# agiger/GPR

Measured on AMD Instinct MI355X. Metric: GP fits/sec (kernel build + Cholesky + solve), N=16384 d=32 fp64, higher is better.
Workload: dtype f64

## Files before the change

gpr_amd/csrc/k_pt_ops.h:

```cpp
#pragma once
#include "k_handoff.h"
#include "k_mma.h"

namespace gprx {
namespace pt {

using namespace mm;
using ho::ld_agent;
using ho::ld_sys;
using ho::ld_uni;
using ho::local_sync;
using ho::publish;
using ho::publish2;
using ho::st_agent;
using ho::st_sys;
using ho::wait_until;
using ho::wave_id;

template <typename T, bool UPDATE, int MAP = 0>
__device__ __forceinline__ void tile_gemm(T* __restrict__ C, int64_t ldc, const T* __restrict__ A, int64_t lda,
                                          const T* __restrict__ B, int64_t ldb, int K, bool lower, T* smem,
                                          const int t, bool tri = false, const uint64_t* Bpan = nullptr) {
    typedef Mfma<T> Tr;
    typedef typename Tr::acc_t acc_t;
    const int lane = t & 63, w = t >> 6;
    int wr, wc;
    wave_block<MAP>(w, wr, wc);
    const int lr = lane & 15, lk = lane >> 4;
    const bool active = !(lower && wr == 0 && wc >= 2);
    T cv[2][4][4];
    if (UPDATE && active) {
#pragma unroll
        for (int x = 0; x < 2; x++)
#pragma unroll
            for (int reg = 0; reg < 4; reg++) {
                const int jl = wc * 32 + x * 16 + Tr::orow(lk, reg);
                const T* ccol = C + (int64_t)jl * ldc;
#pragma unroll
                for (int y = 0; y < 4; y++) cv[x][y][reg] = ccol[wr * 64 + y * 16 + lr];
            }
    }
    acc_t acc[2][4];
    tile_mma<T, MAP>(acc, A, lda, B, ldb, K, !active ? 0 : (tri ? 32 * (wc + 1) : K), smem, t, Bpan);
    if (!active) return;
#pragma unroll
    for (int x = 0; x < 2; x++) {
#pragma unroll
        for (int reg = 0; reg < 4; reg++) {
            const int jl = wc * 32 + x * 16 + Tr::orow(lk, reg);
            T* ccol = C + (int64_t)jl * ldc;
#pragma unroll
            for (int y = 0; y < 4; y++) {
                const int il = wr * 64 + y * 16 + lr;
                if (UPDATE)
                    st_sc1(ccol + il, (lower && il < jl) ? cv[x][y][reg] : cv[x][y][reg] - acc[x][y][reg]);
                else if (!lower || il >= jl)
                    st_sc1(ccol + il, acc[x][y][reg]);
            }
        }
    }
}

template <typename T>
__device__ __forceinline__ void tile_trsm(T* C, int64_t ldc, const T* A, int64_t lda,
                                          const T* __restrict__ B, int64_t ldb, T* smem, const int t) {
    typedef Mfma<T> Tr;
    const int lane = t & 63, w = t >> 6, lr = lane & 15, lk = lane >> 4;
    typename Tr::acc_t acc[2][4];
    mm::tile_mma_trirows<T>(acc, A, lda, B, ldb, smem, t);
#pragma unroll
    for (int x = 0; x < 2; x++)
#pragma unroll
        for (int y = 0; y < 4; y++)
#pragma unroll
            for (int reg = 0; reg < 4; reg++)
                st_sc1(C + (int64_t)(16 * (4 * x + y) + Tr::orow(lk, reg)) * ldc + 16 * w + lr, acc[x][y][reg]);
}

template <typename T>
__device__ __forceinline__ void tile_gemm_rows16(T* __restrict__ C, int64_t ldc, const T* __restrict__ A, int64_t lda,
                                                 const T* __restrict__ B, int64_t ldb, int K, T* smem, const int t) {
    typedef Mfma<T> Tr;
    const int lane = t & 63, w = t >> 6, lr = lane & 15, lk = lane >> 4;
    T cv[4];
#pragma unroll
    for (int reg = 0; reg < 4; reg++) cv[reg] = C[(int64_t)(16 * w + Tr::orow(lk, reg)) * ldc + lr];
    typename Tr::acc_t acc;
    mm::tile_mma_rows16<T>(acc, A, lda, B, ldb, K, smem, t);
#pragma unroll
    for (int reg = 0; reg < 4; reg++) st_sc1(C + (int64_t)(16 * w + Tr::orow(lk, reg)) * ldc + lr, cv[reg] - acc[reg]);
}

template <typename T>
__device__ __forceinline__ void tile_gemm_tall(T* __restrict__ C, int64_t ldc, const T* __restrict__ A, int64_t lda,
                                               const T* __restrict__ B, int64_t ldb, int K, T* smem, const int t) {
    typedef Mfma<T> Tr;
    typedef typename Tr::acc_t acc_t;
    const int lane = t & 63, w = t >> 6;
    const int wr = w & 3, wc = w >> 2, lr = lane & 15, lk = lane >> 4;
    acc_t acc[4][4];
    mm::tile_mma_tall<T, 1>(acc, A, lda, B, ldb, K, smem, t, C, ldc);
#pragma unroll
    for (int x = 0; x < 4; x++)
#pragma unroll
        for (int reg = 0; reg < 4; reg++) {
            T* ccol = C + (int64_t)(64 * wc + 16 * x + Tr::orow(lk, reg)) * ldc;
#pragma unroll
            for (int y = 0; y < 4; y++) st_sc1(ccol + 64 * wr + 16 * y + lr, -acc[x][y][reg]);
        }
}

}
}
```

gpr_amd/csrc/k_ptiles.hip:

```cpp
#include "gprx_dist.h"
#include "gprx_internal.h"
#include "k_handoff.h"
#include "k_pairs.h"
#include "k_pt_diag.h"
#include "k_pt_dist.h"
#include "k_pt_ops.h"
#include "k_pt_split.h"
#include "pt_sched.h"

#include <algorithm>
#include <cstring>
#include <cstdlib>
#include <map>
#include <mutex>
#include <tuple>

namespace gprx {
namespace pt {

template <typename T, int V>
__global__ __launch_bounds__(NT) void diag_bench_kernel(T* A, int64_t ld, T* Linv, int* info, long long* prof,
                                                        int reps) {
    extern __shared__ __attribute__((aligned(16))) unsigned char smem_raw[];
    long long acc[5] = {0, 0, 0, 0, 0};
    long long ph[8] = {0, 0, 0, 0, 0, 0, 0, 0};
    for (int r = 0; r < reps; r++) {
        const long long t0 = wall_clock64();
        if (V == 0) diag_factor_rank8<T>(A + (int64_t)r * DB * ld, ld, Linv, info, 0, smem_raw, threadIdx.x, nullptr, ph);
        else if (V == 1) diag_factor_blocked<T>(A + (int64_t)r * DB * ld, ld, Linv, info, 0, smem_raw, threadIdx.x, ph);
        else diag_factor_la<T>(A + (int64_t)r * DB * ld, ld, Linv, info, 0, smem_raw, threadIdx.x, ph);
        __syncthreads();
        const long long t1 = wall_clock64();
        acc[0] += ph[0];
        acc[1] += ph[1];
        acc[2] += ph[2];
        acc[3] += ph[3];
        acc[4] += t1 - t0;
    }
    if (threadIdx.x == 0) {
        for (int u = 0; u < 5; u++) prof[u] = acc[u];
        for (int u = 0; u < 3; u++) prof[5 + u] = ph[4 + u];
    }
}

template <typename T>
void launch_diag_bench(int variant, T* A, int64_t ld, T* Linv, int* info, long long* prof, int reps, hipStream_t s) {
    const size_t lds = diag_lds<T>() + 64;
    auto go = [&](auto kfn) {
        GPRX_HIP(hipFuncSetAttribute((const void*)kfn, hipFuncAttributeMaxDynamicSharedMemorySize, (int)lds));
        hipLaunchKernelGGL(kfn, dim3(1), dim3(NT), lds, s, A, ld, Linv, info, prof, reps);
    };
    if (variant == 0 || !std::is_same<T, double>::value) go(diag_bench_kernel<T, 0>);
    else if (variant == 1) go(diag_bench_kernel<T, 1>);
    else go(diag_bench_kernel<T, 2>);
    GPRX_HIP(hipGetLastError());
}
template void launch_diag_bench<double>(int, double*, int64_t, double*, int*, long long*, int, hipStream_t);
template void launch_diag_bench<float>(int, float*, int64_t, float*, int*, long long*, int, hipStream_t);

template <typename T>
constexpr size_t pt_lds_bytes() {
    return gemm_lds<T>() > diag_lds<T>() ? gemm_lds<T>() : diag_lds<T>();
}
static_assert(tall_lds<double>() <= pt_lds_bytes<double>() && tall_lds<float>() <= pt_lds_bytes<float>(),
              "the paired update's ring exceeds the LDS of the launch");

template <typename T>
struct Args {
    T* A;
    int64_t ld;
    T* Linv;
    const int4* tasks;
    int ntasks;
    int nc;
    int nv;
    int* ctl;
    int* lcnt;
    int* ver;
    int* info;
    long long tlimit;
    int* dbg;
    int variant;
    long long* trace;
    long long* xt;
    const TileBuild<T>* tb;
    const PtDist<T>* dist;
    int split;
    T* pbuf;
    int* tflag;
    int lab_rows;
};
constexpr int LAB_NARROW = 16;


template <typename T, bool DIST>
__device__ bool wait_inputs(const Args<T>& a, int type, int i, int j, int b0, int nb) {
    const int* vp;
    int vwant;
    const int* vp2;
    int vwant2;
    const int* lp1;
    int lwant1;
    const int* lp2;
    int lwant2;
    const unsigned* rp = nullptr;
    int rn = 0;
    unsigned ep = 0;
    const int* lp3 = nullptr;
    if (type == T_TPART) {
        vp = a.ver + (int64_t)i * a.nv + (i - 1);
        vwant = i - 1;
        vp2 = vp;
        vwant2 = vwant;
        lp1 = a.lcnt + i;
        lwant1 = 0;
        lp2 = lp1;
        lwant2 = 0;
    } else if (type == T_DIAGX && i > 0 && a.split) {
        vp = a.ver + (int64_t)i * a.nv + i;
        vwant = i - 1;
        vp2 = vp;
        vwant2 = vwant;
        lp1 = a.lcnt + i;
        lwant1 = 0;
        lp2 = lp1;
        lwant2 = 0;
    } else if (type == T_DIAGX && i == 0) {
        vp = a.ver;
        vwant = 0;
        vp2 = vp;
        vwant2 = 0;
        lp1 = a.lcnt;
        lwant1 = 0;
        lp2 = lp1;
        lwant2 = 0;
    } else if (type == T_BUILD) {
        return true;
    } else if (type == T_DIAGX) {
        vp = a.ver + (int64_t)i * a.nv + (i - 1);
        vwant = i - 1;
        vp2 = a.ver + (int64_t)i * a.nv + i;
        vwant2 = i - 1;
        lp1 = a.lcnt + (i - 1);
        lwant1 = i;
        lp2 = lp1;
        lwant2 = lwant1;
        if constexpr (DIST) {
            const PtDist<T>& D = *a.dist;
            if (__builtin_amdgcn_readfirstlane(D.loc[i - 1]) < 0) {
                lp1 = lp2 = a.lcnt + i;
                lwant1 = lwant2 = 0;
                rp = dist_flags(D, D.r) + dist_f_linv(D.nr, D.nc) + (i - 1);
                rn = 1;
                ep = D.ep;
            }
        }
    } else if (!DIST && type == T_UPD2) {
        vp = a.ver + (int64_t)i * a.nv + j;
        vwant = b0;
        vp2 = a.ver + (int64_t)(i + 1) * a.nv + j;
        vwant2 = b0;
        lp1 = a.lcnt + i;
        lwant1 = b0 + nb;
        lp2 = a.lcnt + j;
        lwant2 = b0 + nb;
        lp3 = a.lcnt + i + 1;
    } else if (type == T_TRSM) {
        vp = a.ver + (int64_t)i * a.nv + j;
        vwant = j;
        vp2 = vp;
        vwant2 = vwant;
        lp1 = a.lcnt + j;
        lwant1 = j + 1;
        lp2 = lp1;
        lwant2 = lwant1;
        if constexpr (DIST) {
            const PtDist<T>& D = *a.dist;
            if (__builtin_amdgcn_readfirstlane(D.loc[j]) < 0) {
                lp1 = lp2 = a.lcnt + i;
                lwant1 = lwant2 = 0;
                rp = dist_flags(D, D.r) + dist_f_linv(D.nr, D.nc) + j;
                rn = 1;
                ep = D.ep;
            }
        }
    } else {
        const int jc = DIST ? dist_col(a.dist->nc, j) : j;
        vp = a.ver + (int64_t)i * a.nv + jc;
        vwant = b0;
        vp2 = vp;
        vwant2 = vwant;
        lp1 = a.lcnt + i;
        lwant1 = b0 + nb;
        lp2 = a.lcnt + j;
        lwant2 = b0 + nb;
        if constexpr (DIST) {
            const PtDist<T>& D = *a.dist;
            if (__builtin_amdgcn_readfirstlane(D.loc[j]) < 0) {
                lp2 = lp1;
                rp = dist_flags(D, D.r) + dist_f_tile() + (int64_t)j * D.nc + b0;
                rn = nb;
                ep = D.ep;
            }
        }
    }
    const int lane = threadIdx.x & 63;
    const long long t0 = wall_clock64();
    for (;;) {
        int ok = int(ld_uni(vp) == vwant) & int(ld_uni(vp2) == vwant2) & int(ld_uni(lp1) >= lwant1) &
                 int(ld_uni(lp2) >= lwant2);
        if (!DIST && lp3) ok &= int(ld_uni(lp3) >= lwant1);
        if constexpr (DIST) {
            if (rp) {
                const bool good = lane >= rn || ld_sys(rp + (lane < rn ? lane : 0)) == ep;
                ok &= int(__builtin_amdgcn_readfirstlane((uint32_t)(__ballot(!good) == 0)));
            }
        }
        if (ok) return true;
        if (ld_uni(a.ctl + C_ERR)) return false;
        if (wall_clock64() - t0 > a.tlimit) {
            if constexpr (DIST) {
                int miss = int(ld_uni(vp) != vwant) | (int(ld_uni(vp2) != vwant2) << 1) | (int(ld_uni(lp1) < lwant1) << 2) |
                           (int(ld_uni(lp2) < lwant2) << 3);
                int seen = ld_uni(vp);
                if (rp) {
                    const bool good = lane >= rn || ld_sys(rp + (lane < rn ? lane : 0)) == ep;
                    const unsigned long long bad = __ballot(!good);
                    if (bad) {
                        miss |= 16 | ((int)__builtin_ctzll(bad) << 8);
                        seen = (int)__builtin_amdgcn_readfirstlane(ld_sys(rp + (int)__builtin_ctzll(bad)));
                    }
                }
                if (lane == 0) dist_note_timeout(a.dist->check_err + DIST_TO_REC, 1, type, i, j, b0 | (nb << 16), miss, seen);
            }
            st_agent(a.ctl + C_ERR, 1);
            return false;
        }
        __builtin_amdgcn_s_sleep(2);
    }
}

template <typename T>
__device__ __forceinline__ TpCtx<T> tp_ctx(const Args<T>& a) {
    return TpCtx<T>{a.ctl, a.lcnt, a.tflag, a.pbuf, a.dist, a.tlimit, a.xt, a.nc, a.ver, a.nv};
}
template <typename T>
constexpr size_t pt_lds_ctx_off() {
    return pt_lds_bytes<T>() + 16;
}
template <typename T>
constexpr size_t pt_lds_total() {
    return pt_lds_ctx_off<T>() + sizeof(TpCtx<T>);
}

template <typename T, bool DIST>
__global__ __launch_bounds__(NT) void potrf_tiles_kernel(Args<T> a) {
    extern __shared__ __attribute__((aligned(16))) unsigned char smem_raw[];
    int& s_q = *reinterpret_cast<int*>(smem_raw + pt_lds_bytes<T>());
    int& s_ok = *reinterpret_cast<int*>(smem_raw + pt_lds_bytes<T>() + sizeof(int));
    TpCtx<T>* tpc = reinterpret_cast<TpCtx<T>*>(smem_raw + pt_lds_ctx_off<T>());
    if (threadIdx.x == 0) *tpc = tp_ctx(a);
    T* smem = reinterpret_cast<T*>(smem_raw);
    const int t = threadIdx.x;
    const int wv = wave_id();
    const int64_t ld = a.ld;
    for (;;) {
        if (wv == 0) {
            const int v = __hip_atomic_fetch_add(a.ctl + C_TICKET, (t == 0) ? 1 : 0, __ATOMIC_RELAXED,
                                                 __HIP_MEMORY_SCOPE_AGENT);
            s_q = __builtin_amdgcn_readfirstlane(v);
        }
        __syncthreads();
        const int q = __builtin_amdgcn_readfirstlane(s_q);
        if (q >= a.ntasks) break;
        const long long tr0 = a.trace ? wall_clock64() : 0;
        const int4 tk = a.tasks[q];
        const int type = __builtin_amdgcn_readfirstlane(tk.x & 0xff), nb = __builtin_amdgcn_readfirstlane(tk.x >> 8);
        const int i = __builtin_amdgcn_readfirstlane(tk.y), j = __builtin_amdgcn_readfirstlane(tk.z),
                  b0 = __builtin_amdgcn_readfirstlane(tk.w);
        dbg_mark(a.dbg, q, 1 + 10 * type, i, j);
        if (wv == 0) {
            const bool ok0 = wait_inputs<T, DIST>(a, type, i, j, b0, nb);
            if (ok0 && !(a.variant & 32)) {
                bool remote = false;
                if constexpr (DIST) {
                    const PtDist<T>& D = *a.dist;
                    const int dep = (type == T_DIAGX) ? i - 1 : ((type == T_BUILD || type == T_TPART) ? -1 : j);
                    remote = dep >= 0 && __builtin_amdgcn_readfirstlane(D.loc[dep]) < 0 &&
                             !__builtin_amdgcn_readfirstlane(D.acq_agent);
                }
                if (remote) __builtin_amdgcn_fence(__ATOMIC_ACQUIRE, "");
                else __builtin_amdgcn_fence(__ATOMIC_ACQUIRE, "agent");
                asm volatile("s_waitcnt vmcnt(0)" ::: "memory");
            }
            s_ok = ok0 ? 1 : 0;
        }
        __syncthreads();
        if (!__builtin_amdgcn_readfirstlane(s_ok)) break;
        const long long tr1 = a.trace ? wall_clock64() : 0;
        const long long tc1 = a.trace ? (long long)__builtin_amdgcn_s_memtime() : 0;
        dbg_mark(a.dbg, q, 2 + 10 * type, i, j);
        int tid = t;
        asm volatile("" : "+v"(tid));
        if constexpr (DIST) {
            const PtDist<T>& D = *a.dist;
            bool ok = true;
            if (type == T_TPART) {
                ok = tpart_task<T, true>(tpc, dist_tile(a.A, D, i, i - 1), dist_tile(a.A, D, i, i), DB,
                                         a.Linv + (int64_t)(i - 1) * DB * DB, i, j, smem, s_ok, tid);
            } else if (type == T_BUILD) {
                T* tij = dist_tile(a.A, D, i, j);
                const TileBuild<T>& b = *a.tb;
                const bool bad = pr::build_tile_sum<T, 1, true>(
                    b.Kd, b.FU, b.FV, b.nf, b.Kr, b.Kp, b.hd, tij - (int64_t)i * GT - (int64_t)j * GT * DB, DB, b.n,
                    b.sigma2, (int64_t)i * GT, (int64_t)j * GT, smem, tid);
                if (__builtin_amdgcn_readfirstlane(__any(bad))) atomicOr(a.tb->flag, 1);
                publish(a.ver + (int64_t)i * a.nv + j, 0, false);
            } else if (type == T_UPD) {
                const int lj = __builtin_amdgcn_readfirstlane(D.loc[j]);
                const bool loc = lj >= 0;
                const T* Bop = loc ? dist_tile(a.A, D, j, b0) : nullptr;
                const uint64_t* bp = loc ? nullptr : D.tptr + (int64_t)j * D.nc + b0;
                if (D.check && !loc && wv == 0) dist_check_tags(D, j, b0, nb, 0);
                tile_gemm<T, true>(dist_tile(a.A, D, i, j), DB, dist_tile(a.A, D, i, b0), DB, Bop, DB, nb * GT, i == j,
                                   smem, tid, false, bp);
                publish(a.ver + (int64_t)i * a.nv + dist_col(D.nc, j), b0 + nb, false);
                if (D.check && !loc && wv == 0) dist_check_tags(D, j, b0, nb, 1);
                if (!loc && wv == 0) dist_release(D, b0, nb);
            } else if (type == T_TRSM) {
                T* Cik = dist_tile(a.A, D, i, j);
                tile_trsm<T>(Cik, DB, Cik, DB, a.Linv + (int64_t)j * DB * DB, DB, smem, tid);
                publish(a.lcnt + i, j + 1, false);
                if (i == D.nc) {
                    const unsigned all = ((1u << D.g) - 1u) & ~(1u << D.r);
                    dist_push(Cik, D, all, D.o_z + (int64_t)j * DB * DB * (int64_t)sizeof(T),
                              dist_f_tile() + (int64_t)i * D.nc + j, tid);
                } else {
                    const unsigned cm = dist_consumers(D, i);
                    if (wv == 0) ok = dist_wait_release(a, D, cm, j - D.ww);
                    if (wv == 0) s_ok = ok ? 1 : 0;
                    __syncthreads();
                    ok = __builtin_amdgcn_readfirstlane(s_ok) != 0;
                    if (ok)
                        dist_push(Cik, D, cm, -1, dist_f_tile() + (int64_t)i * D.nc + j, tid,
                                  (int64_t)(j % D.ww) * D.nr + i, (D.ep << 16) | (unsigned)(j + 1));
                }
            } else {
                const int k = i;
                T* Akk = dist_tile(a.A, D, k, k);
                T* Akm = k > 0 ? dist_tile(a.A, D, k, k - 1) : nullptr;
                if (k > 0 && a.split) {
                    if constexpr (diag_la<T>) ok = diagx_split<T>(tpc, k, smem, s_ok, tid);
                    else ok = diagx_split_wait<T>(tpc, k, s_ok);
                    if (!ok) break;
                } else if (diag_la<T> && k > 0) {
                    diagx_ts<T>(Akm, Akk, DB, a.Linv + (int64_t)(k - 1) * DB * DB, a.lcnt + k, k, smem, tid, false);
                } else if (k > 0) {
                    tile_trsm<T>(Akm, DB, Akm, DB, a.Linv + (int64_t)(k - 1) * DB * DB, DB, smem, tid);
                    publish(a.lcnt + k, k, false);
                    tile_gemm<T, true, 2>(Akk, DB, Akm, DB, Akm, DB, GT, true, smem, tid);
                    local_sync();
                }
                diag_factor<T>(Akk, DB, a.Linv + (int64_t)k * DB * DB, a.info, (int64_t)k * DB, smem_raw, tid, a.dbg,
                               nullptr, diag_la<T> && k > 0, a.lcnt + k, k + 1);
                const unsigned cm = k > 0 ? dist_consumers(D, k) : 0u;
                const unsigned all = ((1u << D.g) - 1u) & ~(1u << D.r);
                const int nx = (k + 1 < D.nc) ? __builtin_amdgcn_readfirstlane(D.own[k + 1]) : D.r;
                const unsigned first = (nx != D.r) ? (1u << nx) : 0u;
                if (k > 0) {
                    if (wv == 0) ok = dist_wait_release(a, D, cm, k - 1 - D.ww);
                    if (wv == 0) s_ok = ok ? 1 : 0;
                    __syncthreads();
                    ok = __builtin_amdgcn_readfirstlane(s_ok) != 0;
                }
                const int64_t owin = -1;
                const int64_t olinv = D.o_linv + (int64_t)k * DB * DB * (int64_t)sizeof(T);
                const int64_t tix = (int64_t)((k - 1 + D.ww) % D.ww) * D.nr + k;
                const unsigned tgv = (D.ep << 16) | (unsigned)k;
                if (ok && k > 0)
                    dist_push(Akm, D, cm & first, owin, dist_f_tile() + (int64_t)k * D.nc + (k - 1), tid, tix, tgv);
                if (ok) dist_push(a.Linv + (int64_t)k * DB * DB, D, all & first, olinv, dist_f_linv(D.nr, D.nc) + k, tid);
                if (ok && k > 0)
                    dist_push(Akm, D, cm & ~first, owin, dist_f_tile() + (int64_t)k * D.nc + (k - 1), tid, tix, tgv);
                if (ok) dist_push(a.Linv + (int64_t)k * DB * DB, D, all & ~first, olinv, dist_f_linv(D.nr, D.nc) + k, tid);
            }
            if (!ok) break;
        } else {
        T* Ci = a.A + (int64_t)i * GT;
        if (type == T_TPART) {
            (void)tpart_task<T, false>(tpc, Ci + (int64_t)(i - 1) * GT * ld, Ci + (int64_t)i * GT * ld, ld,
                                       a.Linv + (int64_t)(i - 1) * DB * DB, i, j, smem, s_ok, tid);
        } else if (type == T_BUILD) {
            const TileBuild<T>& b = *a.tb;
            const bool bad = pr::build_tile_sum<T, 1, true>(b.Kd, b.FU, b.FV, b.nf, b.Kr, b.Kp, b.hd, a.A, ld, b.n,
                                                            b.sigma2, (int64_t)i * GT, (int64_t)j * GT, smem, tid);
            if (__builtin_amdgcn_readfirstlane(__any(bad))) atomicOr(a.tb->flag, 1);
            publish(a.ver + (int64_t)i * a.nv + j, 0, false);
        } else if (type == T_UPD) {
            const int64_t oa = (a.variant & 64) ? 0 : (int64_t)i * GT + (int64_t)b0 * GT * ld;
            const int64_t ob = (a.variant & 64) ? GT : (int64_t)j * GT + (int64_t)b0 * GT * ld;
            const int64_t lop = (a.variant & 128) ? 0 : ld;
            if (a.variant & 2) {
            } else if (i == a.nc && a.lab_rows <= LAB_NARROW) {
                tile_gemm_rows16<T>(Ci + (int64_t)j * GT * ld, ld, a.A + oa, lop, a.A + ob, lop, nb * GT, smem, tid);
            } else {
                tile_gemm<T, true>(Ci + (int64_t)j * GT * ld, ld, a.A + oa, lop, a.A + ob, lop, nb * GT, i == j, smem,
                                   tid);
            }
            publish(a.ver + (int64_t)i * a.nv + j, b0 + nb, false);
        } else if (type == T_UPD2) {
            if (!(a.variant & 2))
                tile_gemm_tall<T>(Ci + (int64_t)j * GT * ld, ld, a.A + (int64_t)i * GT + (int64_t)b0 * GT * ld, ld,
                                  a.A + (int64_t)j * GT + (int64_t)b0 * GT * ld, ld, nb * GT, smem, tid);
            publish2(a.ver + (int64_t)i * a.nv + j, a.ver + (int64_t)(i + 1) * a.nv + j, b0 + nb);
        } else if (type == T_TRSM) {
            T* Cik = Ci + (int64_t)j * GT * ld;
            if (!(a.variant & 1))
                tile_trsm<T>(Cik, ld, Cik, ld, a.Linv + (int64_t)j * DB * DB, DB, smem, tid);
            publish(a.lcnt + i, j + 1, false);
        } else {
            const int k = i;
            T* Akk = Ci + (int64_t)k * GT * ld;
            long long dt[4] = {0, 0, 0, 0};
            if (k > 0 && a.split) {
                if constexpr (diag_la<T>) (void)diagx_split<T>(tpc, k, smem, s_ok, tid);
                else (void)diagx_split_wait<T>(tpc, k, s_ok);
                if (a.trace) dt[0] = dt[1] = wall_clock64();
            } else if (diag_la<T> && k > 0) {
                T* Akm = Ci + (int64_t)(k - 1) * GT * ld;
                dt[0] = diagx_ts<T>(Akm, Akk, ld, a.Linv + (int64_t)(k - 1) * DB * DB, a.lcnt + k, k, smem, tid,
                                    a.trace != nullptr);
                dt[1] = dt[0];
            } else if (k > 0) {
                T* Akm = Ci + (int64_t)(k - 1) * GT * ld;
                tile_trsm<T>(Akm, ld, Akm, ld, a.Linv + (int64_t)(k - 1) * DB * DB, DB, smem, tid);
                if (a.trace) dt[0] = wall_clock64();
                publish(a.lcnt + k, k, false);
                if (a.trace) dt[1] = wall_clock64();
                tile_gemm<T, true, 2>(Akk, ld, Akm, ld, Akm, ld, GT, true, smem, tid);
                local_sync();
            }
            if (a.trace) dt[2] = wall_clock64();
            diag_factor<T>(Akk, ld, a.Linv + (int64_t)k * DB * DB, a.info, (int64_t)k * DB, smem_raw, tid, a.dbg,
                           a.trace ? a.trace + 4 * (int64_t)(a.ntasks + a.nc) + 4 * (int64_t)k : nullptr,
                           diag_la<T> && k > 0, a.lcnt + k, k + 1);
            if (a.trace) dt[3] = wall_clock64();
            if (a.trace && wv == 0) {
                long long* dp = a.trace + 4 * (int64_t)a.ntasks + 4 * (int64_t)k;
                for (int u = 0; u < 4; u++) dp[u] = dt[u];
            }
        }
        }
        if (a.trace && wv == 0) {
            long long* tp = a.trace + 4 * (int64_t)q;
            tp[0] = tr0;
            tp[1] = tr1;
            tp[2] = wall_clock64();
            tp[3] = (long long)blockIdx.x | (((long long)__builtin_amdgcn_s_memtime() - tc1) << 16);
        }
    }
    dbg_mark(a.dbg, -1, 9, 0, 0);
    if (wv == 0 && ld_agent(a.ctl + C_ERR)) atomicMin(a.info, -1);
}

}

struct PtState {
    struct Dev {
        int4* list = nullptr;
        int64_t n = 0;
        double est_us = 0;
        bool ident_even = false;
        std::vector<int4> host;
    };
    std::map<std::tuple<int, int, bool, int, bool, int>, Dev> sched;
    int* ctr = nullptr;
    void* pbuf = nullptr;
    size_t ctr_ints = 0;
    int ncu = 0;
    int* dbg = nullptr;
    long long* trace = nullptr;
    int64_t trace_n = 0, trace_nc = 0;
    const std::vector<int4>* last_list = nullptr;
    void* tb = nullptr;
    std::vector<unsigned char> tb_last;
    ~PtState() {
        if (tb) (void)hipFree(tb);
        if (pbuf) (void)hipFree(pbuf);
        if (trace) (void)hipFree(trace);
        if (dbg) (void)hipHostFree(dbg);
        for (auto& kv : sched) (void)hipFree(kv.second.list);
        if (ctr) (void)hipFree(ctr);
    }
};

void pt_state_free(PtState* p) { delete p; }

static PtState* g_pt_state = nullptr;
int64_t pt_trace_copy(int32_t* tasks, long long* times, int64_t max) {
    if (!g_pt_state || !g_pt_state->trace || !g_pt_state->last_list) return 0;
    const int64_t n = std::min<int64_t>(max, g_pt_state->trace_n + 7 * g_pt_state->trace_nc);
    GPRX_HIP(hipDeviceSynchronize());
    GPRX_HIP(hipMemcpy(times, g_pt_state->trace, sizeof(long long) * 4 * n, hipMemcpyDeviceToHost));
    const int64_t nl = std::min<int64_t>(n, (int64_t)g_pt_state->last_list->size());
    std::memcpy(tasks, g_pt_state->last_list->data(), sizeof(int4) * nl);
    return n;
}

static int* g_pt_dbg = nullptr;
static int g_pt_dbg_n = 0;
static std::mutex g_pt_dbg_mu;
int pt_debug_snapshot(int* out, int max_wg) {
    std::lock_guard<std::mutex> lk(g_pt_dbg_mu);
    if (!g_pt_dbg) return 0;
    const int n = std::min(max_wg, g_pt_dbg_n);
    for (int k = 0; k < 4 * n; k++) out[k] = __atomic_load_n(g_pt_dbg + k, __ATOMIC_RELAXED);
    return n;
}
void pt_debug_register(int* dbg, int n) {
    std::lock_guard<std::mutex> lk(g_pt_dbg_mu);
    if (n > 0) {
        g_pt_dbg = dbg;
        g_pt_dbg_n = n;
    } else if (g_pt_dbg == dbg) {
        g_pt_dbg = nullptr;
        g_pt_dbg_n = 0;
    }
}

__global__ void pt_init_counters(int* __restrict__ ctr, int64_t n, int64_t v0, int64_t v1) {
    const int64_t i = (int64_t)blockIdx.x * blockDim.x + threadIdx.x;
    if (i < n) ctr[i] = (i >= v0 && i < v1) ? -1 : 0;
}

__global__ void pt_init_identity_counters(int* __restrict__ lcnt, int* __restrict__ ver, int nc, int nr0, int ni,
                                          int even) {
    const int a = blockIdx.x, j = threadIdx.x;
    if (a >= ni) return;
    if (j == 0) lcnt[nr0 + a] = a;
    const int v = even ? a - (a & 1) : a;
    for (int c = j; c < nc; c += blockDim.x) ver[(int64_t)(nr0 + a) * nc + c] = v;
}

template <typename T>
__global__ void pt_init_identity_rows(T* __restrict__ A, int64_t ld, int64_t row0, int64_t nid, int64_t ncol,
                                      int even) {
    const int64_t r = (int64_t)blockIdx.x * blockDim.x + threadIdx.x;
    const int64_t c = blockIdx.y;
    const int64_t rb = r / GT, c0 = (even ? rb - (rb & 1) : rb) * GT;
    if (r >= nid || c >= ncol || c < c0) return;
    A[row0 + r + c * ld] = (r == c) ? T(1) : T(0);
}

template <typename T>
void potrf_tiles(T* A, int64_t ld, int64_t np, int64_t nrows, T* Linv, int* info, Exec& ex, const TileBuild<T>* build,
                 int ni, bool build_only, int lab_live) {
    using namespace pt;
    if (!ex.pt) ex.pt = new PtState();
    PtState& st = *ex.pt;
    if (st.ncu == 0) {
        int dev = 0;
        GPRX_HIP(hipGetDevice(&dev));
        hipDeviceProp_t prop;
        GPRX_HIP(hipGetDeviceProperties(&prop, dev));
        st.ncu = prop.multiProcessorCount;
    }
    GPRX_REQUIRE(np % DB == 0 && nrows % GT == 0 && nrows >= np, GPRX_ERR_ARG, "potrf_tiles: bad sizes");
    const int nc = (int)(np / DB), nr = (int)(nrows / GT);
    const bool fused = build && build->mode != 0;
    GPRX_REQUIRE(ni >= 0 && ni <= nr - nc, GPRX_ERR_ARG, "potrf_tiles: bad identity row blocks");
    GPRX_REQUIRE(!build_only || fused, GPRX_ERR_ARG, "potrf_tiles: build_only needs a fused build");
    const bool split = split_for(std::is_same<T, double>::value, st.ncu);
    const bool narrow = !build_only && lab_live <= LAB_NARROW && nr - ni == nc + 1 && params().label != 0;
    auto key = std::make_tuple(nc, nr, fused, build_only ? -1 : ni, split, (int)sizeof(T) | (narrow ? 256 : 0));
    auto it = st.sched.find(key);
    if (it == st.sched.end()) {
        const Params& pr = params();
        Schedule S;
        if (build_only) {
            for (int i = 0; i < nc; i++)
                for (int j = 0; j <= i; j++) S.list.push_back(make_int4(T_BUILD, i, j, 0));
        } else {
            S = best_schedule(nc, nr, pr, st.ncu, fused, ni, split, std::is_same<T, double>::value, narrow);
        }
        PtState::Dev d;
        d.n = (int64_t)S.list.size();
        d.est_us = S.est_us;
        d.ident_even = S.ident_even;
        GPRX_HIP(dev_malloc(&d.list, sizeof(int4) * std::max<int64_t>(1, d.n)));
        GPRX_HIP(hipMemcpy(d.list, S.list.data(), sizeof(int4) * d.n, hipMemcpyHostToDevice));
        d.host = S.list;
        it = st.sched.emplace(key, d).first;
    }
    const PtState::Dev& sd = it->second;
    const size_t need = (size_t)C_NCTL + nr + (size_t)nr * nc + TP_STRIDE * (size_t)nc;
    if (st.ctr_ints < need) {
        if (st.ctr) GPRX_HIP(hipFree(st.ctr));
        st.ctr = nullptr;
        GPRX_HIP(dev_malloc(&st.ctr, sizeof(int) * need));
        st.ctr_ints = need;
    }
    hipStream_t s = ex.s0;
    {
        const int64_t v0 = fused ? (int64_t)C_NCTL + nr : 0, v1 = fused ? v0 + (int64_t)nc * nc : 0;
        hipLaunchKernelGGL(pt_init_counters, dim3((unsigned)((need + 255) / 256)), dim3(256), 0, s, st.ctr,
                           (int64_t)need, v0, v1);
        GPRX_HIP(hipGetLastError());
    }
    if (ni > 0) {
        hipLaunchKernelGGL(pt_init_identity_counters, dim3((unsigned)ni), dim3(128), 0, s, st.ctr + C_NCTL,
                           st.ctr + C_NCTL + nr, nc, nr - ni, ni, sd.ident_even ? 1 : 0);
        hipLaunchKernelGGL(pt_init_identity_rows<T>, dim3((unsigned)((ni * (int64_t)GT + 255) / 256), (unsigned)np),
                           dim3(256), 0, s, A, ld, (int64_t)(nr - ni) * GT, (int64_t)ni * GT, np, sd.ident_even ? 1 : 0);
    }
    Args<T> a;
    a.A = A;
    a.ld = ld;
    a.Linv = Linv;
    a.tasks = sd.list;
    a.ntasks = (int)sd.n;
    a.nc = nc;
    a.nv = nc;
    a.ctl = st.ctr;
    a.lcnt = st.ctr + C_NCTL;
    a.ver = st.ctr + C_NCTL + nr;
    a.info = info;
    a.tb = nullptr;
    a.dist = nullptr;
    a.split = split ? 1 : 0;
    a.tflag = st.ctr + C_NCTL + nr + (size_t)nr * nc;
    if (split && !st.pbuf) GPRX_HIP(dev_malloc(&st.pbuf, sizeof(T) * 4 * DB * DB));
    a.pbuf = static_cast<T*>(st.pbuf);
    a.lab_rows = narrow ? lab_live : GT;
    if (fused) {
        GPRX_REQUIRE(build->nf == np, GPRX_ERR_ARG, "potrf_tiles: build features must have np rows");
        if (!st.tb) GPRX_HIP(dev_malloc(&st.tb, sizeof(TileBuild<double>)));
        const unsigned char* tbb = reinterpret_cast<const unsigned char*>(build);
        if (st.tb_last.size() != sizeof(TileBuild<T>) || std::memcmp(st.tb_last.data(), tbb, sizeof(TileBuild<T>)) != 0) {
            GPRX_HIP(hipMemcpyAsync(st.tb, build, sizeof(TileBuild<T>), hipMemcpyHostToDevice, s));
            st.tb_last.assign(tbb, tbb + sizeof(TileBuild<T>));
        }
        a.tb = reinterpret_cast<const TileBuild<T>*>(st.tb);
    }
    a.dbg = nullptr;
    a.trace = nullptr;
    a.xt = nullptr;
    static const bool tracing = std::getenv("GPRX_PT_TRACE") != nullptr;
    if (tracing) {
        if (st.trace_n + 7 * st.trace_nc < sd.n + 7 * nc) {
            if (st.trace) GPRX_HIP(hipFree(st.trace));
            GPRX_HIP(dev_malloc(&st.trace, sizeof(long long) * 4 * (sd.n + 7 * nc)));
        }
        st.trace_n = sd.n;
        st.trace_nc = nc;
        a.trace = st.trace;
        a.xt = st.trace + 4 * (sd.n + 2 * nc);
        GPRX_HIP(hipMemsetAsync(a.xt, 0, sizeof(long long) * 4 * 5 * nc, s));
        g_pt_state = &st;
        st.last_list = &sd.host;
    }
    static const int variant = std::getenv("GPRX_PT_VARIANT") ? std::atoi(std::getenv("GPRX_PT_VARIANT")) : 0;
    a.variant = variant;
    static const bool debug = std::getenv("GPRX_PT_DEBUG") != nullptr;
    if (debug) {
        if (!st.dbg) GPRX_HIP(hipHostMalloc((void**)&st.dbg, sizeof(int) * 4 * st.ncu, hipHostMallocCoherent));
        std::memset(st.dbg, 0xff, sizeof(int) * 4 * st.ncu);
        g_pt_dbg = st.dbg;
        g_pt_dbg_n = st.ncu;
        a.dbg = st.dbg;
    }
    a.tlimit = (long long)(1e8 * (2.0 + 20.0 * sd.est_us * 1e-6));
    auto lds_of = [](size_t b) { return std::max<size_t>(b, 96 * 1024); };
    const size_t lds = lds_of(pt_lds_total<T>());
    static bool attr = false;
    if (!attr) {
        GPRX_HIP(hipFuncSetAttribute((const void*)potrf_tiles_kernel<double, false>,
                                     hipFuncAttributeMaxDynamicSharedMemorySize, (int)lds_of(pt_lds_total<double>())));
        GPRX_HIP(hipFuncSetAttribute((const void*)potrf_tiles_kernel<float, false>,
                                     hipFuncAttributeMaxDynamicSharedMemorySize, (int)lds_of(pt_lds_total<float>())));
        attr = true;
    }
    const double nn = (double)np;
    ProfScope ps(KC_TILES, s,
                 nn * nn * nn / 3.0 + (double)(nrows - np - (int64_t)ni * GT) * nn * nn + (ni ? nn * nn * nn / 3.0 : 0.0),
                 0.0);
    hipLaunchKernelGGL((potrf_tiles_kernel<T, false>), dim3((unsigned)st.ncu), dim3(NT), lds, s, a);
    GPRX_HIP(hipGetLastError());
}

template <typename T>
void potrf_tiles_dist_launch(const DistLaunch<T>& L) {
    using namespace pt;
    Args<T> a;
    std::memset(&a, 0, sizeof(a));
    a.A = L.A;
    a.ld = DB;
    a.Linv = L.Linv;
    a.tasks = L.list;
    a.ntasks = L.ntasks;
    a.nc = L.nc;
    a.nv = L.nci;
    a.ctl = L.ctr;
    a.lcnt = L.ctr + C_NCTL;
    a.ver = L.ctr + C_NCTL + L.nr;
    a.info = L.info;
    a.tlimit = L.tlimit;
    a.tb = L.tb_dev;
    a.dist = L.dist_dev;
    a.dbg = L.dbg;
    a.trace = L.trace;
    a.xt = nullptr;
    a.split = L.split;
    a.pbuf = L.pbuf;
    a.tflag = L.tflag;
    a.lab_rows = GT;
    auto lds_of = [](size_t b) { return std::max<size_t>(b, 96 * 1024); };
    const size_t lds = lds_of(pt_lds_total<T>());
    static bool attr = false;
    if (!attr) {
        GPRX_HIP(hipFuncSetAttribute((const void*)potrf_tiles_kernel<double, true>,
                                     hipFuncAttributeMaxDynamicSharedMemorySize, (int)lds_of(pt_lds_total<double>())));
        GPRX_HIP(hipFuncSetAttribute((const void*)potrf_tiles_kernel<float, true>,
                                     hipFuncAttributeMaxDynamicSharedMemorySize, (int)lds_of(pt_lds_total<float>())));
        attr = true;
    }
    hipLaunchKernelGGL((potrf_tiles_kernel<T, true>), dim3((unsigned)L.P), dim3(NT), lds, L.s, a);
    GPRX_HIP(hipGetLastError());
}
template void potrf_tiles_dist_launch<double>(const DistLaunch<double>&);
template void potrf_tiles_dist_launch<float>(const DistLaunch<float>&);

template void potrf_tiles<double>(double*, int64_t, int64_t, int64_t, double*, int*, Exec&, const TileBuild<double>*,
                                  int, bool, int);
template void potrf_tiles<float>(float*, int64_t, int64_t, int64_t, float*, int*, Exec&, const TileBuild<float>*, int,
                                 bool, int);

}
```

Measured before the change: 40.17.

## Prefetch next task ticket during tile stores and unify flag publishing

In the persistent tiled Cholesky kernel, wave 0 now issues the atomic ticket fetch for the next task early, in the middle of the store phase of the UPD, UPD2 and TRSM tile ops, through an inline-asm single-lane atomic. It waits for the result only after the stores, so the next loop iteration can skip its separate ticket atomic and barrier. Dependency-flag publishing is rewritten as one explicit vmcnt drain, a barrier and agent-scope flag stores. The change also adds optional per-stage timestamp tracing. The aim is to hide ticket-dispatch latency behind store traffic, at the cost of inline-asm exec-mask manipulation and a subtler task-claim ordering.

```diff
diff --git a/gpr_amd/csrc/k_pt_ops.h b/gpr_amd/csrc/k_pt_ops.h
--- a/gpr_amd/csrc/k_pt_ops.h
+++ b/gpr_amd/csrc/k_pt_ops.h
@@ -17,10 +17,19 @@
 using ho::wait_until;
 using ho::wave_id;
 
-template <typename T, bool UPDATE, int MAP = 0>
+enum { ST_MFMA = 0, ST_STORES, ST_DRAIN, ST_FLAG, ST_TICKET, ST_DESC, ST_POLL, ST_STAGE0, ST_N };
+struct NoHook {
+    __device__ __forceinline__ void operator()(int) const {}
+};
+__device__ __forceinline__ void stamp(long long* stl, int k) {
+    if (stl && wave_id() == 0) stl[k] = wall_clock64();
+}
+
+template <typename T, bool UPDATE, int MAP = 0, class Pre = NoHook>
 __device__ __forceinline__ void tile_gemm(T* __restrict__ C, int64_t ldc, const T* __restrict__ A, int64_t lda,
                                           const T* __restrict__ B, int64_t ldb, int K, bool lower, T* smem,
-                                          const int t, bool tri = false, const uint64_t* Bpan = nullptr) {
+                                          const int t, bool tri = false, const uint64_t* Bpan = nullptr,
+                                          long long* stl = nullptr, Pre pre = {}) {
     typedef Mfma<T> Tr;
     typedef typename Tr::acc_t acc_t;
     const int lane = t & 63, w = t >> 6;
@@ -42,6 +51,7 @@
     }
     acc_t acc[2][4];
     tile_mma<T, MAP>(acc, A, lda, B, ldb, K, !active ? 0 : (tri ? 32 * (wc + 1) : K), smem, t, Bpan);
+    stamp(stl, ST_MFMA);
     if (!active) return;
 #pragma unroll
     for (int x = 0; x < 2; x++) {
@@ -56,18 +66,24 @@
                     st_sc1(ccol + il, (lower && il < jl) ? cv[x][y][reg] : cv[x][y][reg] - acc[x][y][reg]);
                 else if (!lower || il >= jl)
                     st_sc1(ccol + il, acc[x][y][reg]);
+                if (x == 0 && reg == 0 && y == 0) pre(0);
             }
         }
     }
+    stamp(stl, ST_STORES);
+    pre(1);
 }
 
-template <typename T>
+template <typename T, class Pre = NoHook>
 __device__ __forceinline__ void tile_trsm(T* C, int64_t ldc, const T* A, int64_t lda,
-                                          const T* __restrict__ B, int64_t ldb, T* smem, const int t) {
+                                          const T* __restrict__ B, int64_t ldb, T* smem, const int t,
+                                          long long* stl = nullptr, Pre pre = {}) {
     typedef Mfma<T> Tr;
     const int lane = t & 63, w = t >> 6, lr = lane & 15, lk = lane >> 4;
     typename Tr::acc_t acc[2][4];
     mm::tile_mma_trirows<T>(acc, A, lda, B, ldb, smem, t);
+    stamp(stl, ST_MFMA);
+    pre(0);
 #pragma unroll
     for (int x = 0; x < 2; x++)
 #pragma unroll
@@ -75,11 +91,14 @@
 #pragma unroll
             for (int reg = 0; reg < 4; reg++)
                 st_sc1(C + (int64_t)(16 * (4 * x + y) + Tr::orow(lk, reg)) * ldc + 16 * w + lr, acc[x][y][reg]);
+    stamp(stl, ST_STORES);
+    pre(1);
 }
 
-template <typename T>
+template <typename T, class Pre = NoHook>
 __device__ __forceinline__ void tile_gemm_rows16(T* __restrict__ C, int64_t ldc, const T* __restrict__ A, int64_t lda,
-                                                 const T* __restrict__ B, int64_t ldb, int K, T* smem, const int t) {
+                                                 const T* __restrict__ B, int64_t ldb, int K, T* smem, const int t,
+                                                 long long* stl = nullptr, Pre pre = {}) {
     typedef Mfma<T> Tr;
     const int lane = t & 63, w = t >> 6, lr = lane & 15, lk = lane >> 4;
     T cv[4];
@@ -87,19 +106,28 @@
     for (int reg = 0; reg < 4; reg++) cv[reg] = C[(int64_t)(16 * w + Tr::orow(lk, reg)) * ldc + lr];
     typename Tr::acc_t acc;
     mm::tile_mma_rows16<T>(acc, A, lda, B, ldb, K, smem, t);
+    stamp(stl, ST_MFMA);
 #pragma unroll
-    for (int reg = 0; reg < 4; reg++) st_sc1(C + (int64_t)(16 * w + Tr::orow(lk, reg)) * ldc + lr, cv[reg] - acc[reg]);
+    for (int reg = 0; reg < 4; reg++) {
+        st_sc1(C + (int64_t)(16 * w + Tr::orow(lk, reg)) * ldc + lr, cv[reg] - acc[reg]);
+        if (reg == 0) pre(0);
+    }
+    stamp(stl, ST_STORES);
+    pre(1);
 }
 
-template <typename T>
+template <typename T, class Pre = NoHook>
 __device__ __forceinline__ void tile_gemm_tall(T* __restrict__ C, int64_t ldc, const T* __restrict__ A, int64_t lda,
-                                               const T* __restrict__ B, int64_t ldb, int K, T* smem, const int t) {
+                                               const T* __restrict__ B, int64_t ldb, int K, T* smem, const int t,
+                                               long long* stl = nullptr, Pre pre = {}) {
     typedef Mfma<T> Tr;
     typedef typename Tr::acc_t acc_t;
     const int lane = t & 63, w = t >> 6;
     const int wr = w & 3, wc = w >> 2, lr = lane & 15, lk = lane >> 4;
     acc_t acc[4][4];
     mm::tile_mma_tall<T, 1>(acc, A, lda, B, ldb, K, smem, t, C, ldc);
+    stamp(stl, ST_MFMA);
+    pre(0);
 #pragma unroll
     for (int x = 0; x < 4; x++)
 #pragma unroll
@@ -108,6 +136,8 @@
 #pragma unroll
             for (int y = 0; y < 4; y++) st_sc1(ccol + 64 * wr + 16 * y + lr, -acc[x][y][reg]);
         }
+    stamp(stl, ST_STORES);
+    pre(1);
 }
 
 }
diff --git a/gpr_amd/csrc/k_ptiles.hip b/gpr_amd/csrc/k_ptiles.hip
--- a/gpr_amd/csrc/k_ptiles.hip
+++ b/gpr_amd/csrc/k_ptiles.hip
@@ -89,6 +89,7 @@
     T* pbuf;
     int* tflag;
     int lab_rows;
+    int overlap;
 };
 constexpr int LAB_NARROW = 16;
 
@@ -246,7 +247,7 @@
 }
 template <typename T>
 constexpr size_t pt_lds_ctx_off() {
-    return pt_lds_bytes<T>() + 16;
+    return pt_lds_bytes<T>() + 32 + sizeof(long long) * (ST_N + 1);
 }
 template <typename T>
 constexpr size_t pt_lds_total() {
@@ -258,19 +259,24 @@
     extern __shared__ __attribute__((aligned(16))) unsigned char smem_raw[];
     int& s_q = *reinterpret_cast<int*>(smem_raw + pt_lds_bytes<T>());
     int& s_ok = *reinterpret_cast<int*>(smem_raw + pt_lds_bytes<T>() + sizeof(int));
+    long long* s_st = reinterpret_cast<long long*>(smem_raw + pt_lds_bytes<T>() + 32);
     TpCtx<T>* tpc = reinterpret_cast<TpCtx<T>*>(smem_raw + pt_lds_ctx_off<T>());
     if (threadIdx.x == 0) *tpc = tp_ctx(a);
     T* smem = reinterpret_cast<T*>(smem_raw);
     const int t = threadIdx.x;
     const int wv = wave_id();
     const int64_t ld = a.ld;
+    bool pre = false;
     for (;;) {
-        if (wv == 0) {
-            const int v = __hip_atomic_fetch_add(a.ctl + C_TICKET, (t == 0) ? 1 : 0, __ATOMIC_RELAXED,
-                                                 __HIP_MEMORY_SCOPE_AGENT);
-            s_q = __builtin_amdgcn_readfirstlane(v);
-        }
-        __syncthreads();
+        if (!pre) {
+            if (wv == 0) {
+                const int v = __hip_atomic_fetch_add(a.ctl + C_TICKET, (t == 0) ? 1 : 0, __ATOMIC_RELAXED,
+                                                     __HIP_MEMORY_SCOPE_AGENT);
+                s_q = __builtin_amdgcn_readfirstlane(v);
+                if (!DIST && a.trace) s_st[ST_TICKET] = wall_clock64();
+            }
+            __syncthreads();
+        }
         const int q = __builtin_amdgcn_readfirstlane(s_q);
         if (q >= a.ntasks) break;
         const long long tr0 = a.trace ? wall_clock64() : 0;
@@ -279,8 +285,15 @@
         const int i = __builtin_amdgcn_readfirstlane(tk.y), j = __builtin_amdgcn_readfirstlane(tk.z),
                   b0 = __builtin_amdgcn_readfirstlane(tk.w);
         dbg_mark(a.dbg, q, 1 + 10 * type, i, j);
+        long long* stl = (!DIST && a.trace) ? s_st : nullptr;
+        if (stl && wv == 0) {
+            if (pre) s_st[ST_TICKET] = s_st[ST_N];
+            s_st[ST_DESC] = wall_clock64();
+            s_st[ST_MFMA] = s_st[ST_STORES] = s_st[ST_DRAIN] = s_st[ST_FLAG] = s_st[ST_STAGE0] = 0;
+        }
         if (wv == 0) {
             const bool ok0 = wait_inputs<T, DIST>(a, type, i, j, b0, nb);
+            if (stl) s_st[ST_POLL] = wall_clock64();
             if (ok0 && !(a.variant & 32)) {
                 bool remote = false;
                 if constexpr (DIST) {
@@ -387,6 +400,27 @@
             if (!ok) break;
         } else {
         T* Ci = a.A + (int64_t)i * GT;
+        int* pf1 = nullptr;
+        int* pf2 = nullptr;
+        int pv = 0;
+        int cv = 0, cq = 0;
+        bool cl = false;
+        auto claim = [&](int ph) {
+            if (a.overlap && wv == 0) {
+                if (ph == 0) {
+                    unsigned long long keep;
+                    asm volatile(
+                        "s_nop 4\n\ts_mov_b64 %1, exec\n\ts_mov_b64 exec, 1\n\tglobal_atomic_add %0, %2, %3, %4 sc0\n\t"
+                        "s_mov_b64 exec, %1"
+                        : "=&v"(cv), "=&s"(keep)
+                        : "v"(0), "v"(1), "s"(a.ctl + C_TICKET)
+                        : "memory");
+                } else {
+                    asm volatile("s_waitcnt vmcnt(0)" : "+v"(cv)::"memory");
+                    cq = __builtin_amdgcn_readfirstlane(cv);
+                }
+            }
+        };
         if (type == T_TPART) {
             (void)tpart_task<T, false>(tpc, Ci + (int64_t)(i - 1) * GT * ld, Ci + (int64_t)i * GT * ld, ld,
                                        a.Linv + (int64_t)(i - 1) * DB * DB, i, j, smem, s_ok, tid);
@@ -395,29 +429,40 @@
             const bool bad = pr::build_tile_sum<T, 1, true>(b.Kd, b.FU, b.FV, b.nf, b.Kr, b.Kp, b.hd, a.A, ld, b.n,
                                                             b.sigma2, (int64_t)i * GT, (int64_t)j * GT, smem, tid);
             if (__builtin_amdgcn_readfirstlane(__any(bad))) atomicOr(a.tb->flag, 1);
-            publish(a.ver + (int64_t)i * a.nv + j, 0, false);
+            pf1 = pf2 = a.ver + (int64_t)i * a.nv + j;
         } else if (type == T_UPD) {
             const int64_t oa = (a.variant & 64) ? 0 : (int64_t)i * GT + (int64_t)b0 * GT * ld;
             const int64_t ob = (a.variant & 64) ? GT : (int64_t)j * GT + (int64_t)b0 * GT * ld;
             const int64_t lop = (a.variant & 128) ? 0 : ld;
             if (a.variant & 2) {
             } else if (i == a.nc && a.lab_rows <= LAB_NARROW) {
-                tile_gemm_rows16<T>(Ci + (int64_t)j * GT * ld, ld, a.A + oa, lop, a.A + ob, lop, nb * GT, smem, tid);
+                tile_gemm_rows16<T>(Ci + (int64_t)j * GT * ld, ld, a.A + oa, lop, a.A + ob, lop, nb * GT, smem, tid,
+                                    stl, claim);
+                cl = true;
             } else {
                 tile_gemm<T, true>(Ci + (int64_t)j * GT * ld, ld, a.A + oa, lop, a.A + ob, lop, nb * GT, i == j, smem,
-                                   tid);
-            }
-            publish(a.ver + (int64_t)i * a.nv + j, b0 + nb, false);
+                                   tid, false, nullptr, stl, claim);
+                cl = true;
+            }
+            pf1 = pf2 = a.ver + (int64_t)i * a.nv + j;
+            pv = b0 + nb;
         } else if (type == T_UPD2) {
-            if (!(a.variant & 2))
+            if (!(a.variant & 2)) {
                 tile_gemm_tall<T>(Ci + (int64_t)j * GT * ld, ld, a.A + (int64_t)i * GT + (int64_t)b0 * GT * ld, ld,
-                                  a.A + (int64_t)j * GT + (int64_t)b0 * GT * ld, ld, nb * GT, smem, tid);
-            publish2(a.ver + (int64_t)i * a.nv + j, a.ver + (int64_t)(i + 1) * a.nv + j, b0 + nb);
+                                  a.A + (int64_t)j * GT + (int64_t)b0 * GT * ld, ld, nb * GT, smem, tid, stl, claim);
+                cl = true;
+            }
+            pf1 = a.ver + (int64_t)i * a.nv + j;
+            pf2 = a.ver + (int64_t)(i + 1) * a.nv + j;
+            pv = b0 + nb;
         } else if (type == T_TRSM) {
             T* Cik = Ci + (int64_t)j * GT * ld;
-            if (!(a.variant & 1))
-                tile_trsm<T>(Cik, ld, Cik, ld, a.Linv + (int64_t)j * DB * DB, DB, smem, tid);
-            publish(a.lcnt + i, j + 1, false);
+            if (!(a.variant & 1)) {
+                tile_trsm<T>(Cik, ld, Cik, ld, a.Linv + (int64_t)j * DB * DB, DB, smem, tid, stl, claim);
+                cl = true;
+            }
+            pf1 = pf2 = a.lcnt + i;
+            pv = j + 1;
         } else {
             const int k = i;
             T* Akk = Ci + (int64_t)k * GT * ld;
@@ -450,6 +495,23 @@
                 for (int u = 0; u < 4; u++) dp[u] = dt[u];
             }
         }
+        pre = false;
+        if (pf1) {
+            cl = cl && a.overlap != 0;
+            if (cl && wv == 0) {
+                if (stl) stl[ST_N] = wall_clock64();
+                s_q = cq;
+            }
+            asm volatile("s_waitcnt vmcnt(0)" ::: "memory");
+            stamp(stl, ST_DRAIN);
+            __syncthreads();
+            if (wv == 0) {
+                st_agent(pf1, pv);
+                if (pf2 != pf1) st_agent(pf2, pv);
+                if (stl) stl[ST_FLAG] = wall_clock64();
+            }
+            pre = cl;
+        }
         }
         if (a.trace && wv == 0) {
             long long* tp = a.trace + 4 * (int64_t)q;
@@ -457,6 +519,10 @@
             tp[1] = tr1;
             tp[2] = wall_clock64();
             tp[3] = (long long)blockIdx.x | (((long long)__builtin_amdgcn_s_memtime() - tc1) << 16);
+            if constexpr (!DIST) {
+                long long* xs = a.trace + 4 * ((int64_t)a.ntasks + 7 * (int64_t)a.nc) + ST_N * (int64_t)q;
+                for (int u = 0; u < ST_N; u++) xs[u] = s_st[u];
+            }
         }
     }
     dbg_mark(a.dbg, -1, 9, 0, 0);
@@ -499,7 +565,7 @@
 static PtState* g_pt_state = nullptr;
 int64_t pt_trace_copy(int32_t* tasks, long long* times, int64_t max) {
     if (!g_pt_state || !g_pt_state->trace || !g_pt_state->last_list) return 0;
-    const int64_t n = std::min<int64_t>(max, g_pt_state->trace_n + 7 * g_pt_state->trace_nc);
+    const int64_t n = std::min<int64_t>(max, 3 * g_pt_state->trace_n + 7 * g_pt_state->trace_nc);
     GPRX_HIP(hipDeviceSynchronize());
     GPRX_HIP(hipMemcpy(times, g_pt_state->trace, sizeof(long long) * 4 * n, hipMemcpyDeviceToHost));
     const int64_t nl = std::min<int64_t>(n, (int64_t)g_pt_state->last_list->size());
@@ -632,6 +698,8 @@
     if (split && !st.pbuf) GPRX_HIP(dev_malloc(&st.pbuf, sizeof(T) * 4 * DB * DB));
     a.pbuf = static_cast<T*>(st.pbuf);
     a.lab_rows = narrow ? lab_live : GT;
+    static const int overlap = std::getenv("GPRX_PT_OVERLAP") ? std::atoi(std::getenv("GPRX_PT_OVERLAP")) : 1;
+    a.overlap = overlap;
     if (fused) {
         GPRX_REQUIRE(build->nf == np, GPRX_ERR_ARG, "potrf_tiles: build features must have np rows");
         if (!st.tb) GPRX_HIP(dev_malloc(&st.tb, sizeof(TileBuild<double>)));
@@ -647,9 +715,9 @@
     a.xt = nullptr;
     static const bool tracing = std::getenv("GPRX_PT_TRACE") != nullptr;
     if (tracing) {
-        if (st.trace_n + 7 * st.trace_nc < sd.n + 7 * nc) {
+        if (3 * st.trace_n + 7 * st.trace_nc < 3 * sd.n + 7 * nc) {
             if (st.trace) GPRX_HIP(hipFree(st.trace));
-            GPRX_HIP(dev_malloc(&st.trace, sizeof(long long) * 4 * (sd.n + 7 * nc)));
+            GPRX_HIP(dev_malloc(&st.trace, sizeof(long long) * 4 * (3 * sd.n + 7 * nc)));
         }
         st.trace_n = sd.n;
         st.trace_nc = nc;
```

Result: no change. 40.41, median of 6 (+0.6%).
